# UCSD-Comp-Imaging/Nerf-Simple

Hardware: NVIDIA B200
Metric: rays/sec (64 samples/ray) render (higher is better)
Workload: dtype bf16

## Files before the change

nerf_simple_b200/csrc/mlp_chain.cuh:

```cuda
constexpr uint32_t kC_A = 0, kC_E = 2 * kABytes, kC_W = kC_E + 2 * kEBytes;
constexpr int kCStages = 4;
constexpr uint32_t kCStageBytes = 16384;
constexpr uint32_t kC_Bar = kC_W + kCStages * kCStageBytes;
constexpr uint32_t kC_Bias = kC_Bar + 256;
constexpr uint32_t kCSmemLaunch = kC_Bias + 2 * 1024;
constexpr int kCThreads = 640;
constexpr int kCProducerWarp = 16, kCMmaWarp = 17, kCStoreWarp0 = 18;
constexpr uint32_t kB_WFull = 0, kB_WPeer = 32, kB_WEmpty = 64, kB_Act = 96, kB_Acc = 112, kB_Tmem = 128, kB_Written = 136,
                   kB_StoreFree = 152;

struct TileCtx {
  int64_t tile;
  int slot;
  int half;
  int part;
  uint32_t r;
  uint32_t rowoff;
  uint32_t r7s;
  uint32_t a_img, e_img, t_lane;
  uint32_t b_img;
  const float* gf;
};
__device__ __forceinline__ uint32_t sw_off(const TileCtx& c, uint32_t kb, uint32_t j) {
  return kb * 16384u + c.rowoff + ((j << 4) ^ c.r7s);
}

__device__ __forceinline__ void slot_barrier(int slot) {
  asm volatile("bar.sync %0, 256;" ::"r"(slot + 1) : "memory");
}

#ifdef NB200_DEV
constexpr bool kDevBuild = true;
#else
constexpr bool kDevBuild = false;
#endif
struct SlabC { int src, kb, n, ksteps, both_a; };
constexpr int kSchedFwd = 0, kSchedBwd = 1, kSchedFwd3 = 2, kSchedFwdFold = 3;
constexpr int kSchedBwd3 = 4;
__host__ __device__ constexpr int sched_fwd_slabs(int l) { return l == 0 ? 1 : ((l == 5 || l == 9) ? 5 : 4); }
__host__ __device__ constexpr SlabC sched_fwd_slab(int l, int s) {
  return l == 0 ? SlabC{1, 0, 256, 4, 0}
                : (l == 9 ? (s < 4 ? SlabC{0, s, 128, 4, 0} : SlabC{1, 0, 128, 2, 0})
                          : (s < 4 ? SlabC{0, s, 256, 4, 0} : SlabC{1, 0, 256, 4, 0}));
}
template <int kSched> __host__ __device__ constexpr bool sched_is_bwd() { return kSched == kSchedBwd || kSched == kSchedBwd3; }
template <int kSched> __host__ __device__ constexpr int sched_slabs(int l) {
  return kSched == kSchedBwd3 ? 2 * (l == 0 ? 2 : 4)
         : kSched == kSchedFwd ? sched_fwd_slabs(l)
                             : (kSched == kSchedFwdFold ? sched_fwd_slabs(l >= 8 ? 9 : l) : (kSched == kSchedBwd ? (l == 0 ? 2 : 4) : 2 * sched_fwd_slabs(l)));
}
template <int kSched> __host__ __device__ constexpr SlabC sched_slab(int l, int s) {
  if (kSched == kSchedFwd) return sched_fwd_slab(l, s);
  if (kSched == kSchedFwdFold) return sched_fwd_slab(l >= 8 ? 9 : l, s);
  if (kSched == kSchedBwd) return SlabC{0, s, 256, 4, 0};
  if (kSched == kSchedBwd3) return SlabC{0, s >> 1, 256, 4, (s & 1) ? 0 : 1};
  SlabC c = sched_fwd_slab(l, s >> 1);
  c.both_a = (s & 1) ? 0 : 1;
  return c;
}

struct MmaRing { uint32_t stage, phase; };

template <int kSched> __host__ __device__ constexpr int sched_class_rep(int l) {
  return sched_is_bwd<kSched>() ? (l == 0 ? 0 : 1) : ((l == 0 || l == 5 || l == 9) ? l : ((kSched == kSchedFwdFold && l == 8) ? 9 : 1));
}

template <class Epi, int L, int S>
__device__ __forceinline__ void issue_slab(uint32_t smem_base, uint32_t bar, uint32_t tmem_base, uint64_t desc_hi, uint32_t slot,
                                           bool replay, bool release, MmaRing& r) {
  constexpr SlabC sc = sched_slab<Epi::kSched>(L, S);
  constexpr int NS = sched_slabs<Epi::kSched>(L);
  if (!replay) {
    mbar_wait(bar + kB_WFull + 8 * r.stage, r.phase, 400);
    tc_fence_after();
  }
  const uint32_t a_addr = smem_base + (sc.src ? kC_E + slot * kEBytes : kC_A + slot * kABytes + (uint32_t)sc.kb * 16384u);
  const uint64_t adesc = desc_hi | (uint64_t)((a_addr >> 4) & 0x3FFFu);
  const uint64_t bdesc = desc_hi | (uint64_t)(((smem_base + kC_W + r.stage * kCStageBytes) >> 4) & 0x3FFFu);
  constexpr uint32_t idesc = umma_idesc_bf16(256, sc.n, 0, 0);
// ... 96 lines not shown
    c.half = (warp >> 2) & 1;
    c.part = warp >> 2;
    c.r = (uint32_t)(warp & 3) * 32u + (uint32_t)lane;
    c.rowoff = c.r * 128u;
    c.r7s = (c.r & 7u) << 4;
    c.a_img = smem_base + kC_A + slot * kABytes;
    c.e_img = smem_base + kC_E + slot * kEBytes;
    c.t_lane = tmem_base + (((uint32_t)(warp & 3) * 32u) << 16) + (uint32_t)slot * 256u;
    c.b_img = smem_base + kC_Bias + (uint32_t)slot * 1024u;
    c.gf = reinterpret_cast<const float*>(p.packed + (Epi::kSched == kSchedFwd3 || Epi::kSched == kSchedBwd3 ? c_layout.f32_off3 : c_layout.f32_off));
    const uint32_t act_remote = mapa_shared(bar + kB_Act + 8 * slot, 0);
    uint32_t acc_parity = 0, free_parity = 0;
    typename Epi::State st;
    bool first_step = true;
    long long t_epi = 0, t_accw = 0, t_pro = 0, t_reclaim = 0, t_after = 0, t_stage = 0;
    auto publish = [&](bool to_mma) {
      fence_proxy_async_smem();
      tc_fence_before();
      __syncwarp();
      if (lane == 0) {
        if (Epi::kBulkStore) mbar_arrive(bar + kB_Written + 8 * slot);
        if (to_mma) mbar_arrive_cluster(act_remote);
      }
    };
    const uint32_t bias_t = threadIdx.x & 255u;
    auto fetch_bias = [&](int l) -> float { return Epi::kStageBias ? __ldg(c.gf + kF32Bias + Epi::bias_row(l) * 256 + (int)bias_t) : 0.f; };
    auto stage_bias = [&](float v) {
      if (!Epi::kStageBias) return;
      if (Epi::kSlots == 2) slot_barrier(slot); else asm volatile("bar.sync 1, 512;" ::: "memory");
      if (Epi::kSlots == 2 || threadIdx.x < 256u) asm volatile("st.shared.f32 [%0], %1;" ::"r"(c.b_img + bias_t * 4u), "f"(v) : "memory");
      if (Epi::kSlots == 2) slot_barrier(slot); else asm volatile("bar.sync 1, 512;" ::: "memory");
    };
    auto reclaim = [&]() {
      if (Epi::kBulkStore && !first_step) {
        mbar_wait(bar + kB_StoreFree + 8 * slot, free_parity, 500);
        free_parity ^= 1;
      }
      first_step = false;
    };
    Epi::init_slot(c);
    for (int64_t k = slot; k < my_pt; k += Epi::kSlots) {
      c.tile = 2 * (cid + k * C) + rank;
      if (Epi::kReverseTiles) c.tile = 2 * (PT - 1 - (cid + k * C)) + rank;
      reclaim();
      long long tq0 = 0;
      if constexpr (Epi::kHasDbg && kDevBuild) tq0 = clock64();
      const float bias0 = fetch_bias(0);
      Epi::begin_tile(p, st, c);
      publish(true);
      stage_bias(bias0);
      if constexpr (Epi::kHasDbg && kDevBuild) t_pro += clock64() - tq0;
      for (int l = 0; l < Epi::kNumLayers; ++l) {
        Epi::prefetch(p, st, c, l);
        if constexpr (Epi::kHasDbg && kDevBuild) tq0 = clock64();
        mbar_wait(bar + kB_Acc + 8 * slot, acc_parity, 100 + l);
        acc_parity ^= 1;
        tc_fence_after();
        long long tq1 = 0;
        if constexpr (Epi::kHasDbg && kDevBuild) { tq1 = clock64(); t_accw += tq1 - tq0; }
        reclaim();
        if constexpr (Epi::kHasDbg && kDevBuild) t_reclaim += clock64() - tq1;
        const float bias_next = fetch_bias(l + 1 < Epi::kNumLayers ? l + 1 : l);
        Epi::layer(p, st, c, l);
        if (Epi::kBulkStore || l + 1 < Epi::kNumLayers) publish(l + 1 < Epi::kNumLayers);
        if constexpr (Epi::kHasDbg && kDevBuild) {
          const long long tq2 = clock64();
          t_epi += tq2 - tq1;
          if ((p.dbg & 8) && threadIdx.x == 0 && rank == 0 && p.dbg_counters) {
            atomicAdd(p.dbg_counters + 16 + l, (unsigned long long)(tq2 - tq1));
            atomicAdd(p.dbg_counters + 32 + l, (unsigned long long)(tq1 - tq0));
          }
        }
        long long tq3 = 0;
        if constexpr (Epi::kHasDbg && kDevBuild) tq3 = clock64();
        if (l + 1 < Epi::kNumLayers) stage_bias(bias_next);
        long long tq4 = 0;
        if constexpr (Epi::kHasDbg && kDevBuild) { tq4 = clock64(); t_stage += tq4 - tq3; }
        Epi::after_publish(p, st, c, l);
        if constexpr (Epi::kHasDbg && kDevBuild) t_after += clock64() - tq4;
      }
    }
    if constexpr (Epi::kHasDbg && kDevBuild) {
      if ((p.dbg & 8) && threadIdx.x == 0 && rank == 0 && p.dbg_counters) {
        atomicAdd(p.dbg_counters + 4, (unsigned long long)t_epi);
        atomicAdd(p.dbg_counters + 5, (unsigned long long)t_accw);
        atomicAdd(p.dbg_counters + 6, (unsigned long long)t_pro);
        atomicAdd(p.dbg_counters + 12, (unsigned long long)t_reclaim);
        atomicAdd(p.dbg_counters + 13, (unsigned long long)t_stage);
        atomicAdd(p.dbg_counters + 14, (unsigned long long)t_after);
      }
    }
    if (Epi::kBulkStore && !first_step) mbar_wait(bar + kB_StoreFree + 8 * slot, free_parity, 501);
  } else if (warp == kCProducerWarp) {
    if (lane == 0) {
      uint32_t stage = 0, phase = 0;
      long long t_pempty = 0;
      for (int64_t pr = 0; pr * Epi::kSlots < my_pt; ++pr) {
        const int nslots = (Epi::kSlots == 2 && my_pt - 2 * pr >= 2) ? 2 : 1;
        int s0 = 0;
        for (int l = 0; l < Epi::kNumLayers; ++l) {
          int s1 = s0;
          while (!slabs[s1].last) ++s1;
          const int reps = (nslots == 2 && s1 - s0 + 1 <= kCStages) ? 1 : nslots;
          for (int rep = 0; rep < reps; ++rep) {
// ... 105 lines not shown
  float f;
  int64_t ray_begin;
};
constexpr int kInCamera = 2;

__device__ __forceinline__ void load_ray_chain(const FwdEpiParams& p, int64_t ray, float (&o)[6]) {
  if (p.in_mode == kInCamera) {
    camera_ray(p.poses, p.H, p.W, p.f, p.ray_begin + ray, o);
  } else {
    const float2* q = reinterpret_cast<const float2*>(p.in0 + ray * 6);
    const float2 a = __ldg(q), b = __ldg(q + 1), c = __ldg(q + 2);
    o[0] = a.x; o[1] = a.y; o[2] = b.x; o[3] = b.y; o[4] = c.x; o[5] = c.y;
  }
}

template <bool kRender>
__device__ __forceinline__ void load_query_chain(const FwdEpiParams& p, int64_t m, float v[6], float& t) {
  if (!kRender && p.in_mode == NB200_IN_POINTS) {
    const float2* q = reinterpret_cast<const float2*>(p.in0 + m * 6);
    const float2 a = __ldg(q), b = __ldg(q + 1), c = __ldg(q + 2);
    v[0] = a.x; v[1] = a.y; v[2] = b.x; v[3] = b.y; v[4] = c.x; v[5] = c.y;
    t = 0.f;
  } else {
    const int64_t ray = p.nshift >= 0 ? (m >> p.nshift) : m / p.N;
    float o[6];
    if (kRender) {
      load_ray_chain(p, ray, o);
      t = p.sampler ? philox_sample_depth(m, (int)(m - ray * p.N), p.N, p.tn, p.tf, p.seed, p.offset) : __ldg(p.in1 + m);
    } else {
      const float2* q = reinterpret_cast<const float2*>(p.in0 + ray * 6);
      const float2 a = __ldg(q), b = __ldg(q + 1), c = __ldg(q + 2);
      o[0] = a.x; o[1] = a.y; o[2] = b.x; o[3] = b.y; o[4] = c.x; o[5] = c.y;
      t = __ldg(p.in1 + m);
    }
    const float dx = o[3], dy = o[4], dz = o[5];
    v[0] = __fadd_rn(o[0], __fmul_rn(dx, t));
    v[1] = __fadd_rn(o[1], __fmul_rn(dy, t));
    v[2] = __fadd_rn(o[2], __fmul_rn(dz, t));
    const float inv = 1.0f / sqrtf(fmaf(dz, dz, fmaf(dy, dy, dx * dx)));
    v[3] = dx * inv; v[4] = dy * inv; v[5] = dz * inv;
  }
}

template <int S>
__device__ __forceinline__ void composite_staged_ray(const FwdEpiParams& p, uint32_t stage_o, uint32_t stage_t, int ray_local,
                                                     int64_t ray, int lane) {
  constexpr int N = 32 * S;
  float4 o[S];
  float t[S];
  const uint32_t row0 = (uint32_t)(ray_local * N + lane * S);
#pragma unroll
  for (int j = 0; j < S; ++j) {
    asm volatile("ld.shared.v4.f32 {%0,%1,%2,%3}, [%4];" : "=f"(o[j].x), "=f"(o[j].y), "=f"(o[j].z), "=f"(o[j].w) : "r"(stage_o + (row0 + j) * 16u));
    asm volatile("ld.shared.f32 %0, [%1];" : "=f"(t[j]) : "r"(stage_t + (row0 + j) * 4u));
  }
// ... 115 lines not shown
    load_bias16(c, cbase + (q + 1) * 16, bq);
    tmem_ld_wait();
    if (q + 2 < 8) tmem_ld16(c.t_lane + cbase + (q + 2) * 16, a0);
    epi_cols16<kRelu, kSigma, kSave>(c, a1, cbase + (q + 1) * 16, bq, sigma);
  }
}
template <bool kRelu, bool kSigma, bool kSave>
__device__ __forceinline__ void epi_hidden(const TileCtx& c, float& sigma) {
  if (c.half == 0) epi_hidden_h<kRelu, kSigma, kSave, 0>(c, sigma);
  else epi_hidden_h<kRelu, kSigma, kSave, 1>(c, sigma);
}
#ifdef NB_PROBE_NOLDTM
#undef tmem_ld16
#endif

template <bool kSave, bool kRender = false, bool kFold = false>
struct FwdEpi {
  static_assert(!(kSave && kRender), "the fused render kernel is inference only");
  using Params = FwdEpiParams;
  static constexpr bool kHasDbg = true;
  static constexpr bool kBulkStore = kSave;
  static constexpr int kSched = kFold ? kSchedFwdFold : kSchedFwd;
  static constexpr bool kStageBias = true;
  static constexpr int kSlots = 2;
  static constexpr int kNumLayers = kFold ? kNumFoldLayers : kNumMmaLayers;
  static constexpr bool kReverseTiles = false;
  __device__ static constexpr int ml_of(int l) { return (kFold && l == 8) ? 9 : l; }
  __device__ static constexpr int bias_row(int l) { return (kFold && l == 8) ? kFoldBiasRow : l; }
  struct State {
    float v[6];
    float sigma;
    float t;
    int64_t m_raw;
    bool row_valid;
  };
  __device__ static const SlabDesc* slabs() { return kFold ? c_layout.fwdf : c_layout.fwd; }
  __device__ static void init_slot(const TileCtx&) {}

  __device__ static void prefetch(const Params&, State&, const TileCtx&, int) {}

  __device__ static void after_publish(const Params& p, State& st, const TileCtx& c, int l) {
    const int ml = ml_of(l);
    if (ml == 5) {
      if (c.half == 0) encode_row<kLd, 0, 2>(st.v + 3, c.e_img, c.r, nullptr);
      else encode_row<kLd, 2, 4>(st.v + 3, c.e_img, c.r, nullptr);
#pragma unroll
      for (uint32_t i = threadIdx.x & 255u; i < kTabFloats; i += 256u) {
        const float v = __ldg(c.gf + (i < kTabWC1 ? kF32WSig + (int)i
                                                  : (i < kTabBC1 ? kF32WC1 + (int)(i - kTabWC1) : (i < kTabBSig ? kF32BC1 + (int)(i - kTabBC1) : kF32BSig))));
        asm volatile("st.shared.f32 [%0], %1;" ::"r"(c.e_img + tab_off(i)), "f"(v) : "memory");
      }
    }
    if (!kSave || ml < 0 || ml == 8) return;
    const int64_t T = p.num_tiles;
    if (ml < 8) {
      uint8_t* row = p.saved + mask_tensor_off(ml, T) + (size_t)c.tile * 4096 + ((size_t)(c.half * 128) + c.r) * 16;
      uint32_t m[4];
#pragma unroll
      for (int q = 0; q < 4; ++q) {
        const uint32_t kb = (uint32_t)(c.half * 2 + (q >> 1)), j0 = (uint32_t)(q & 1) * 4u;
// ... 19 lines not shown
          uint32_t w0, w1, w2, w3;
          asm volatile("ld.shared.v4.b32 {%0,%1,%2,%3}, [%4];" : "=r"(w0), "=r"(w1), "=r"(w2), "=r"(w3)
                       : "r"(c.a_img + sw_off(c, (uint32_t)c.half, (uint32_t)(q * 4 + j))));
          add_pair_flags(f[j >> 1], w0, 4 * (j & 1)); add_pair_flags(f[j >> 1], w1, 4 * (j & 1) + 1);
          add_pair_flags(f[j >> 1], w2, 4 * (j & 1) + 2); add_pair_flags(f[j >> 1], w3, 4 * (j & 1) + 3);
        }
        m[q] = fold_mask16(f[0]) | (fold_mask16(f[1]) << 16);
      }
      *reinterpret_cast<uint2*>(row) = make_uint2(m[0], m[1]);
    }
  }

  __device__ static void begin_tile(const Params& p, State& st, const TileCtx& c) {
    st.m_raw = c.tile * kTileM + c.r;
    st.row_valid = st.m_raw < p.M;
    load_query_chain<kRender>(p, st.row_valid ? st.m_raw : p.M - 1, st.v, st.t);
    st.sigma = 0.f;
    if (c.half == 0) encode_row<kLp, 0, 4>(st.v, c.e_img, c.r, nullptr);
    else encode_row<kLp, 4, 8>(st.v, c.e_img, c.r, nullptr);
  }

  __device__ static void store_tile(const Params& p, const TileCtx& c, int l) {
    const int64_t T = p.num_tiles;
    const int ml = ml_of(l);
    if (ml == -1) tma_bulk_s2g(p.saved + saved_tensor_off(10, T) + (size_t)c.tile * 16384, c.e_img, 16384);
    else if (ml < 9) tma_bulk_s2g(p.saved + saved_tensor_off(ml, T) + (size_t)c.tile * 65536, c.a_img, 65536);
    else tma_bulk_s2g(p.saved + saved_tensor_off(9, T) + (size_t)c.tile * 32768, c.a_img, 32768);
    if (ml == 6) tma_bulk_s2g(p.saved + saved_tensor_off(11, T) + (size_t)c.tile * 16384, c.e_img, 16384);
  }

  __device__ static void layer(const Params& p, State& st, const TileCtx& c, int l) {
    const int ml = ml_of(l);
    if (ml < 9) {
      if (ml == 7) epi_hidden<true, true, kSave>(c, st.sigma);
      else if (ml == 8) epi_hidden<false, false, kSave>(c, st.sigma);
      else epi_hidden<true, false, kSave>(c, st.sigma);
    } else {
      float rgb[3] = {0.f, 0.f, 0.f};
#pragma unroll 1
      for (int q = 0; q < 2; ++q) {
        const int col0 = c.half * 64 + q * 32;
        uint32_t a[32];
        tmem_ld32(c.t_lane + col0, a);
        tmem_ld_wait();
#pragma unroll
        for (int j = 0; j < 4; ++j) {
          float x[8], b[8];
          asm volatile("ld.shared.v4.f32 {%0,%1,%2,%3}, [%4];" : "=f"(b[0]), "=f"(b[1]), "=f"(b[2]), "=f"(b[3]) : "r"(c.b_img + (uint32_t)(col0 + 8 * j) * 4u));
          asm volatile("ld.shared.v4.f32 {%0,%1,%2,%3}, [%4];" : "=f"(b[4]), "=f"(b[5]), "=f"(b[6]), "=f"(b[7]) : "r"(c.b_img + (uint32_t)(col0 + 8 * j + 4) * 4u));
#pragma unroll
          for (int e = 0; e < 8; ++e) x[e] = fmaxf(__uint_as_float(a[8 * j + e]) + b[e], 0.f);
#pragma unroll
          for (int k = 0; k < 3; ++k) {
            const float4 w0 = tab_ld4(c.e_img, kTabWC1 + (uint32_t)(k * 128 + col0 + 8 * j)), w1 = tab_ld4(c.e_img, kTabWC1 + (uint32_t)(k * 128 + col0 + 8 * j + 4));
            rgb[k] = fmaf(x[0], w0.x, rgb[k]); rgb[k] = fmaf(x[1], w0.y, rgb[k]); rgb[k] = fmaf(x[2], w0.z, rgb[k]); rgb[k] = fmaf(x[3], w0.w, rgb[k]);
            rgb[k] = fmaf(x[4], w1.x, rgb[k]); rgb[k] = fmaf(x[5], w1.y, rgb[k]); rgb[k] = fmaf(x[6], w1.z, rgb[k]); rgb[k] = fmaf(x[7], w1.w, rgb[k]);
          }
          if (kSave) {
            const uint32_t w0 = pack_bf16x2(x[0], x[1]), w1 = pack_bf16x2(x[2], x[3]), w2 = pack_bf16x2(x[4], x[5]),
                           w3 = pack_bf16x2(x[6], x[7]);
            st_shared_v4(c.a_img + sw_off(c, (uint32_t)c.half, (uint32_t)(q * 4 + j)), w0, w1, w2, w3);
          }
        }
      }
// ... 53 lines not shown
#pragma unroll
    for (int e = 0; e < 4; ++e) split_hi_lo(f[8 * j + 2 * e], f[8 * j + 2 * e + 1], h[e], l[e]);
    st_shared_v4(img_hi + sw128_off(r, j), h[0], h[1], h[2], h[3]);
    st_shared_v4(img_lo + sw128_off(r, j), l[0], l[1], l[2], l[3]);
  }
}

__device__ __forceinline__ uint32_t relu_bit(int col_in_step) { return 1u << ((col_in_step >> 1) + 8 * (col_in_step & 1)); }

template <bool kSave>
struct FwdEpi3 {
  using Params = FwdEpiParams;
  static constexpr bool kHasDbg = false;
  static constexpr bool kBulkStore = kSave;
  static constexpr int kSched = kSchedFwd3;
  static constexpr bool kStageBias = true;
  static constexpr int kSlots = 1;
  static constexpr int kNumLayers = kNumMmaLayers;
  static constexpr bool kReverseTiles = false;
  struct State {
    float v[6];
    float sigma;
    int64_t m_raw;
    bool row_valid;
  };
  __device__ static const SlabDesc* slabs() { return c_layout.fwd3; }
  __device__ static constexpr int bias_row(int l) { return l; }
  __device__ static void init_slot(const TileCtx&) {}
  __device__ static void prefetch(const Params&, State&, const TileCtx&, int) {}
  __device__ static void after_publish(const Params&, State&, const TileCtx&, int) {}
// ... 142 lines not shown
      asm volatile("bar.sync 1, 512;" ::: "memory");
    }
  }
};

#ifndef NB_DG_L2HINT
#define NB_DG_L2HINT 2
#endif
template <bool kFold>
struct DgradEpi {
  using Params = BwdParams;
  static constexpr bool kHasDbg = false;
  static constexpr bool kBulkStore = true;
  static constexpr int kSched = kSchedBwd;
  static constexpr bool kStageBias = false;
  static constexpr int kSlots = 2;
  static constexpr int kNumLayers = kFold ? 8 : 9;
  static constexpr int kBl0 = kFold ? 2 : 1;
  static constexpr bool kReverseTiles = true;
  struct State { float4 g; uint4 mask; };
  __device__ static const SlabDesc* slabs() { return kFold ? c_layout.bwdf : c_layout.bwd; }
  __device__ static constexpr int bias_row(int l) { return l; }
  __device__ static void after_publish(const Params&, State&, const TileCtx&, int) {}
  __device__ static void init_slot(const TileCtx& c) {
    for (uint32_t i = threadIdx.x & 255u; i < 640u; i += 256u)
      asm volatile("st.shared.f32 [%0], %1;" ::"r"(c.e_img + i * 4u), "f"(__ldg(c.gf + (i < 256u ? kF32WSig + (int)i : kF32WC1 + (int)(i - 256u)))) : "memory");
    slot_barrier(c.slot);
  }
  __device__ static __forceinline__ float4 head_ld4(const TileCtx& c, uint32_t i) {
    float4 v;
// ... 93 lines not shown

  __device__ static void layer(const Params&, State& st, const TileCtx& c, int l) {
    const int bl = l + kBl0;
    if (bl == 1) layer_t<false, false>(st, c);
    else if (bl == 2) layer_t<true, true>(st, c);
    else layer_t<true, false>(st, c);
  }
};

struct DgradEpi3 {
  using Params = BwdParams;
  static constexpr bool kHasDbg = false;
  static constexpr bool kBulkStore = true;
  static constexpr int kSched = kSchedBwd3;
  static constexpr bool kStageBias = false;
  static constexpr int kSlots = 1;
  static constexpr int kNumLayers = 9;
  static constexpr bool kReverseTiles = true;
  struct State { float4 g; uint2 mask; };
  __device__ static const SlabDesc* slabs() { return c_layout.bwd3; }
  __device__ static constexpr int bias_row(int l) { return l; }
  __device__ static void after_publish(const Params&, State&, const TileCtx&, int) {}
  __device__ static void init_slot(const TileCtx& c) {
    for (uint32_t i = threadIdx.x; i < 640u; i += 512u)
      asm volatile("st.shared.f32 [%0], %1;" ::"r"(c.e_img + i * 4u), "f"(__ldg(c.gf + (i < 256u ? kF32WSig + (int)i : kF32WC1 + (int)(i - 256u)))) : "memory");
    asm volatile("bar.sync 1, 512;" ::: "memory");
  }
  __device__ static __forceinline__ float4 head_ld4(const TileCtx& c, uint32_t i) {
    float4 v;
    asm volatile("ld.shared.v4.f32 {%0,%1,%2,%3}, [%4];" : "=f"(v.x), "=f"(v.y), "=f"(v.z), "=f"(v.w) : "r"(c.e_img + i * 4u));
// ... 90 lines not shown
```

nerf_simple_b200/csrc/mlp_tc.cu:

```cuda
#include <cuda.h>
#include <stdlib.h>
#include <string.h>

#include <mutex>
#include <type_traits>
#include <utility>

#include "common.cuh"
#include "stream_common.cuh"
#include "tc_common.cuh"

namespace nb200 {
using namespace tc;

constexpr int kNumMmaLayers = 10;
constexpr int kMaxSlabs = 48;
constexpr int kNumFoldLayers = kNumMmaLayers - 1;
constexpr int kLayerFold = 100;
constexpr int kFoldBiasRow = 10;

struct SlabDesc {
  uint32_t off;
  uint32_t bytes;
  uint16_t n;
// ... 21 lines not shown
  SlabDesc bwd[kMaxSlabs];
  int num_fwdf;
  SlabDesc fwdf[kMaxSlabs];
  int num_bwdf;
  SlabDesc bwdf[kMaxSlabs];
  int num_fold;
  SlabDesc fold[8];
  uint32_t f32_off;
  uint32_t total_bytes;
  int num_fwd3;
  SlabDesc fwd3[2 * kMaxSlabs];
  uint32_t f32_off3;
  uint32_t total_bytes3;
  int num_bwd3;
  SlabDesc bwd3[2 * kMaxSlabs];
};
constexpr int kF32Bias = 0, kF32WSig = 2816, kF32BSig = 3072, kF32WC1 = 3076, kF32BC1 = 3460,
              kF32Floats = 3520;
constexpr int kF32Wf = kF32Floats, kF32WgT = kF32Wf + 128 * 256, kF32Wc0g = kF32WgT + 256 * 256, kF32Bg = kF32Wc0g + 128 * 256,
              kF32FloatsFold = kF32Bg + 256;

__constant__ __align__(16) PackedLayout c_layout;
static PackedLayout h_layout;
static bool h_layout_built = false;

constexpr int kMaxDevices = 64;
struct DeviceState { bool layout_uploaded, attr_fwd, attr_render, attr_bwd, attr_x3, attr_bwd3; int arch; };
static DeviceState g_dev[kMaxDevices];
static std::mutex g_mu;
static int current_device(int* dev) {
// ... 57 lines not shown
  }
  h_layout.num_bwd = t.s;
  LayoutBuilder f;
  f.arr = h_layout.fold; f.off = t.off; f.s = 0;
  for (int kb = 0; kb < 4; ++kb) f.add(9, kLayerFold, 0, 128, kb * 64, 64, kHidden, 0, kb, 4);
  for (int kb = 0; kb < 2; ++kb) f.add(2, kLayerFold, 1, 256, kb * 64, 64, kHidden, 0, kb, 4);
  h_layout.num_fold = f.s;
  {
    int n = 0;
    for (int i = 0; i < h_layout.num_fwd; ++i)
      if (h_layout.fwd[i].ml < 8) h_layout.fwdf[n++] = h_layout.fwd[i];
    for (int kb = 0; kb < 4; ++kb) h_layout.fwdf[n++] = h_layout.fold[kb];
    h_layout.fwdf[n - 4].first = 1;
    h_layout.fwdf[n++] = h_layout.fwd[h_layout.num_fwd - 1];
    h_layout.num_fwdf = n;
    n = 0;
    for (int kb = 0; kb < 2; ++kb) h_layout.bwdf[n++] = h_layout.fold[4 + kb];
    h_layout.bwdf[0].first = 1; h_layout.bwdf[1].last = 1;
    for (int i = 0; i < h_layout.num_bwd; ++i)
      if (h_layout.bwd[i].ml >= 3) h_layout.bwdf[n++] = h_layout.bwd[i];
    h_layout.num_bwdf = n;
  }
  h_layout.f32_off = f.off;
  h_layout.total_bytes = f.off + kF32FloatsFold * (uint32_t)sizeof(float);
  LayoutBuilder x;
  x.arr = h_layout.fwd3; x.off = 0; x.s = 0;
  for (int i = 0; i < h_layout.num_fwd; ++i) {
    const SlabDesc& f = h_layout.fwd[i];
    for (int lo = 0; lo < 2; ++lo) {
      x.add(f.ml, f.layer, 0, f.n, f.wcol0, f.kvalid, f.ldw, f.src, f.kb, f.ksteps, lo, lo ? 0 : 1);
// ... 193 lines not shown
__host__ __device__ __forceinline__ size_t mask_tensor_off(int t, int64_t num_tiles) {
  return (kSavedDataTileBytes + (size_t)t * 4096) * (size_t)num_tiles;
}
__host__ __device__ __forceinline__ size_t saved_tensor_off(int t, int64_t num_tiles) {
  const size_t per_tile = t < 9 ? (size_t)t * 65536 : (t == 9 ? 9 * 65536 : (t == 10 ? 9 * 65536 + 32768 : 9 * 65536 + 49152));
  return per_tile * (size_t)num_tiles;
}
__host__ __device__ __forceinline__ size_t saved_tile_bytes(int t) {
  return t < 9 ? 65536 : (t == 9 ? 32768 : 16384);
}
constexpr size_t kSavedTileBytes3 = 2 * kSavedDataTileBytes + kMaskTileBytes;
__host__ __device__ __forceinline__ size_t mask_tensor_off3(int t, int64_t num_tiles) {
  return (2 * kSavedDataTileBytes + (size_t)t * 4096) * (size_t)num_tiles;
}

template <int L, int J0, int J1>
__device__ __forceinline__ void encode_row(const float* x, uint32_t img_base, uint32_t r, uint8_t* gsave) {
  float f[64];
#pragma unroll
  for (int i = 0; i < 64; ++i) f[i] = 0.f;
#pragma unroll
  for (int c = 0; c < 3; ++c) {
    f[c] = x[c];
    float s, co;
    sincosf(x[c], &s, &co);
#pragma unroll
    for (int i = 0; i < L; ++i) {
      f[3 + c * 2 * L + 2 * i] = s;
      f[3 + c * 2 * L + 2 * i + 1] = co;
      const float s2 = 2.f * s * co;
      co = fmaf(-2.f * s, s, 1.f);
      s = s2;
    }
  }
#pragma unroll
  for (int j = J0; j < J1; ++j) {
    const uint32_t w0 = pack_bf16x2(f[8 * j], f[8 * j + 1]), w1 = pack_bf16x2(f[8 * j + 2], f[8 * j + 3]),
                   w2 = pack_bf16x2(f[8 * j + 4], f[8 * j + 5]), w3 = pack_bf16x2(f[8 * j + 6], f[8 * j + 7]);
    st_shared_v4(img_base + sw128_off(r, j), w0, w1, w2, w3);
    if (gsave) *reinterpret_cast<uint4*>(gsave + sw128_off(r, j)) = make_uint4(w0, w1, w2, w3);
  }
}

#include "mlp_tc_bwd.cuh"
#include "mlp_chain.cuh"

template <int kSched>
static bool schedule_matches(const SlabDesc* tab, int num, int layers) {
  int i = 0;
// ... 2 lines not shown
    for (int k = 0; k < ns; ++k, ++i) {
      if (i >= num) return false;
      const SlabC c = sched_slab<kSched>(l, k);
      const SlabDesc& d = tab[i];
      if (d.src != c.src || d.kb != c.kb || d.n != c.n || d.ksteps != c.ksteps || ((d.flags & kSlabBothA) != 0) != (c.both_a != 0) ||
          (d.first != 0) != (k == 0) || (d.last != 0) != (k == ns - 1) || d.bytes != (uint32_t)c.n * 128u)
        return false;
    }
  }
  return i == num;
}
static bool check_schedules() {
  return schedule_matches<kSchedFwd>(h_layout.fwd, h_layout.num_fwd, kNumMmaLayers) &&
         schedule_matches<kSchedBwd>(h_layout.bwd, h_layout.num_bwd, 9) &&
         schedule_matches<kSchedFwdFold>(h_layout.fwdf, h_layout.num_fwdf, kNumFoldLayers) &&
         schedule_matches<kSchedBwd>(h_layout.bwdf, h_layout.num_bwdf, 8) &&
         schedule_matches<kSchedFwd3>(h_layout.fwd3, h_layout.num_fwd3, kNumMmaLayers) &&
         schedule_matches<kSchedBwd3>(h_layout.bwd3, h_layout.num_bwd3, 9);
}

size_t tc_packed_bytes(int x3) {
  std::lock_guard<std::mutex> lock(g_mu);
  ensure_host_layout();
  return x3 ? h_layout.total_bytes3 : h_layout.total_bytes;
}
static int64_t train_tiles(int64_t M) { return (ceil_div64(M, kTileM) + 1) & ~(int64_t)1; }
size_t tc_saved_bytes(int64_t M) { return (size_t)train_tiles(M) * kSavedTileBytes; }
constexpr int kPadPitchWide = 320, kPadPitchX = 64;
constexpr size_t kPadC0 = 0, kPadSkip = kPadC0 + 128 * kPadPitchWide, kPadL00 = kPadSkip + 256 * kPadPitchWide,
                 kPadFoldS = kPadL00 + 256 * kPadPitchX,
// ... 139 lines not shown
}

int tc_forward(int in_mode, const float* in0, const float* in1, int64_t M, int N, const void* packed,
               float* out, void* saved, void*, size_t, int fold, cudaStream_t s) {
  NB_TRY_RC(check_arch());
  NB_TRY_RC(ensure_layout());
  NB_TRY_RC(ensure_attr(&DeviceState::attr_fwd, []() -> int {
    NB_CUDA_CHECK(cudaFuncSetAttribute(chain_kernel<FwdEpi<false>>, cudaFuncAttributeMaxDynamicSharedMemorySize,
                                       (int)kCSmemLaunch));
    NB_CUDA_CHECK(cudaFuncSetAttribute(chain_kernel<FwdEpi<true>>, cudaFuncAttributeMaxDynamicSharedMemorySize,
                                       (int)kCSmemLaunch));
    NB_CUDA_CHECK(cudaFuncSetAttribute(chain_kernel<FwdEpi<false, false, true>>, cudaFuncAttributeMaxDynamicSharedMemorySize,
                                       (int)kCSmemLaunch));
    NB_CUDA_CHECK(cudaFuncSetAttribute(chain_kernel<FwdEpi<true, false, true>>, cudaFuncAttributeMaxDynamicSharedMemorySize,
                                       (int)kCSmemLaunch));
    return NB200_OK;
  }));
  const int64_t T = saved ? train_tiles(M) : ceil_div64(M, kTileM);
  FwdEpiParams p;
  TmapPair tm;
  NB_TRY_RC(get_tmaps(packed, &tm));
  p.tmap128 = tm.m128; p.tmap64 = tm.m64;
  p.dbg = 0;
  p.dbg_counters = nullptr;
#ifdef NB200_DEV
  { const char* e = getenv("NB200_DBG"); p.dbg = e ? atoi(e) : 0; }
  if (p.dbg & 8) {
    static unsigned long long* ctr = nullptr;
    if (!ctr) { cudaMalloc(&ctr, 512); cudaMemset(ctr, 0, 512); }
    unsigned long long h[64];
    cudaMemcpy(h, ctr, 512, cudaMemcpyDeviceToHost);
    printf("nb200 dbg: mma-warp cycles wait_act=%llu total=%llu | epilogue warp 0: layers=%llu wait_acc=%llu prologue=%llu | producer wait_empty=%llu | epilogue warp 0: reclaim (inside layers)=%llu stage_bias=%llu after_publish=%llu\n",
           h[0], h[3], h[4], h[5], h[6], h[7], h[12], h[13], h[14]);
    printf("nb200 dbg: epilogue warp 0 per layer, busy | wait_acc (share of total):");
    for (int l = 0; l < 10; ++l) printf(" L%d %.1f|%.1f", l, 100.0 * (double)h[16 + l] / (double)(h[3] ? h[3] : 1), 100.0 * (double)h[32 + l] / (double)(h[3] ? h[3] : 1));
    printf("\n");
    cudaMemset(ctr, 0, 512);
    p.dbg_counters = ctr;
  }
#endif
  p.in_mode = in_mode; p.in0 = in0; p.in1 = in1; p.M = M; p.N = N;
  p.nshift = (N > 0 && (N & (N - 1)) == 0) ? __builtin_ctz((unsigned)N) : -1;
  p.packed = reinterpret_cast<const uint8_t*>(packed);
  p.out = out; p.saved = reinterpret_cast<uint8_t*>(saved);
  p.num_tiles = T;
  const int grid = chain_grid(T);
  if (saved && fold)
    chain_kernel<FwdEpi<true, false, true>><<<grid, kCThreads, kCSmemLaunch, s>>>(p);
  else if (saved)
    chain_kernel<FwdEpi<true>><<<grid, kCThreads, kCSmemLaunch, s>>>(p);
  else if (fold)
    chain_kernel<FwdEpi<false, false, true>><<<grid, kCThreads, kCSmemLaunch, s>>>(p);
  else
    chain_kernel<FwdEpi<false>><<<grid, kCThreads, kCSmemLaunch, s>>>(p);
  NB_LAUNCH_CHECK("chain_kernel<FwdEpi>");
  return NB200_OK;
}

static int chain_grid_x3(int64_t T) {
  const int64_t PT = (T + 1) / 2, maxc = sm_count() / 2;
  return (int)(2 * (PT < maxc ? PT : maxc));
}

int tc_forward_x3(int in_mode, const float* in0, const float* in1, int64_t M, int N, const void* packed, float* out,
                  void* saved, cudaStream_t s) {
// ... 21 lines not shown
  else chain_kernel<FwdEpi3<false>><<<grid, kCThreads, kCSmemLaunch, s>>>(p);
  NB_LAUNCH_CHECK("chain_kernel<FwdEpi3>");
  return NB200_OK;
}

int tc_render(const float* rays, const float* poses, int H, int W, float f, int64_t ray_begin, const float* ts, uint64_t seed,
              uint64_t offset, int64_t B, int N, float tn, float tf, const void* packed, float* rgb, float* disp, float* acc,
              int fold, cudaStream_t s) {
  NB_TRY_RC(check_arch());
  NB_TRY_RC(ensure_layout());
  NB_TRY_RC(ensure_attr(&DeviceState::attr_render, []() -> int {
    NB_CUDA_CHECK(cudaFuncSetAttribute(chain_kernel<FwdEpi<false, true>>, cudaFuncAttributeMaxDynamicSharedMemorySize,
                                       (int)kCSmemLaunch));
    NB_CUDA_CHECK(cudaFuncSetAttribute(chain_kernel<FwdEpi<false, true, true>>, cudaFuncAttributeMaxDynamicSharedMemorySize,
                                       (int)kCSmemLaunch));
    return NB200_OK;
  }));
  const int64_t M = B * N, T = ceil_div64(M, kTileM);
  FwdEpiParams p;
  memset(&p, 0, sizeof(p));
  TmapPair tm;
  NB_TRY_RC(get_tmaps(packed, &tm));
  p.tmap128 = tm.m128; p.tmap64 = tm.m64;
  p.in_mode = rays ? NB200_IN_RAYS : kInCamera; p.in0 = rays; p.in1 = ts; p.M = M; p.N = N;
  p.nshift = (N > 0 && (N & (N - 1)) == 0) ? __builtin_ctz((unsigned)N) : -1;
  p.packed = reinterpret_cast<const uint8_t*>(packed);
  p.num_tiles = T;
  p.rgb = rgb; p.disp = disp; p.acc = acc; p.B = B;
  p.sampler = ts ? 0 : 1; p.seed = seed; p.offset = offset; p.tn = tn; p.tf = tf;
  p.poses = poses; p.H = H; p.W = W; p.f = f; p.ray_begin = ray_begin;
  if (fold) chain_kernel<FwdEpi<false, true, true>><<<chain_grid(T), kCThreads, kCSmemLaunch, s>>>(p);
  else chain_kernel<FwdEpi<false, true>><<<chain_grid(T), kCThreads, kCSmemLaunch, s>>>(p);
  NB_LAUNCH_CHECK("chain_kernel<FwdEpi<render>>");
  return NB200_OK;
}

static void wgrad_item(WItem& w, const uint8_t* ds, const uint8_t* sv, int64_t T, float* pad, float* const* G, int dt, int st,
                       int layer, int ldw, int col0, int ncols, int nrows, bool bias) {
  w.a_ptr = ds + delta_tensor_off(dt, T);
  w.a_tile_bytes = dt == 0 ? 32768u : 65536u;
  w.a_chunks = dt == 0 ? 2 : 4;
  w.b_ptr = sv + saved_tensor_off(st, T);
  w.b_tile_bytes = (uint32_t)saved_tile_bytes(st);
  w.b_chunks = st >= 10 ? 1 : 4;
  w.n_mma = st >= 10 ? 64 : 256;
  w.dW = G[2 * layer]; w.db = bias ? G[2 * layer + 1] : nullptr;
// ... 171 lines not shown
```

Measured before the change: 20.03 million.

## Fold per-ray view-direction term into colour-layer bias for folded inference

Adds a ray-bias mode for the folded forward chain. Within a tile all samples share a ray direction, so the view-direction encoding's contribution to the colour layer is computed once per ray in scalar code and added to the bias. That drops the extra K-slab MMA and the direction encoding per sample. It also prefetches the next tile's ray and t values during the last layer in the non-render path, and adds debug timing for tile boundaries. In exchange the bias is now per ray, with two rays per 128-row tile when N is 64. The path is limited to N of 64 or 128, and the dot product is done on CUDA cores with bf16-rounded inputs.

```diff
diff --git a/nerf_simple_b200/csrc/mlp_chain.cuh b/nerf_simple_b200/csrc/mlp_chain.cuh
--- a/nerf_simple_b200/csrc/mlp_chain.cuh
+++ b/nerf_simple_b200/csrc/mlp_chain.cuh
@@ -19,6 +19,8 @@
   uint32_t r7s;
   uint32_t a_img, e_img, t_lane;
   uint32_t b_img;
+  bool first_tile;
+  int64_t next_tile;
   const float* gf;
 };
 __device__ __forceinline__ uint32_t sw_off(const TileCtx& c, uint32_t kb, uint32_t j) {
@@ -37,6 +39,7 @@
 struct SlabC { int src, kb, n, ksteps, both_a; };
 constexpr int kSchedFwd = 0, kSchedBwd = 1, kSchedFwd3 = 2, kSchedFwdFold = 3;
 constexpr int kSchedBwd3 = 4;
+constexpr int kSchedFwdRay = 5;
 __host__ __device__ constexpr int sched_fwd_slabs(int l) { return l == 0 ? 1 : ((l == 5 || l == 9) ? 5 : 4); }
 __host__ __device__ constexpr SlabC sched_fwd_slab(int l, int s) {
   return l == 0 ? SlabC{1, 0, 256, 4, 0}
@@ -47,11 +50,13 @@
 template <int kSched> __host__ __device__ constexpr int sched_slabs(int l) {
   return kSched == kSchedBwd3 ? 2 * (l == 0 ? 2 : 4)
          : kSched == kSchedFwd ? sched_fwd_slabs(l)
+         : kSched == kSchedFwdRay ? (l >= 8 ? 4 : sched_fwd_slabs(l))
                              : (kSched == kSchedFwdFold ? sched_fwd_slabs(l >= 8 ? 9 : l) : (kSched == kSchedBwd ? (l == 0 ? 2 : 4) : 2 * sched_fwd_slabs(l)));
 }
 template <int kSched> __host__ __device__ constexpr SlabC sched_slab(int l, int s) {
   if (kSched == kSchedFwd) return sched_fwd_slab(l, s);
   if (kSched == kSchedFwdFold) return sched_fwd_slab(l >= 8 ? 9 : l, s);
+  if (kSched == kSchedFwdRay) return l >= 8 ? SlabC{0, s, 128, 4, 0} : sched_fwd_slab(l, s);
   if (kSched == kSchedBwd) return SlabC{0, s, 256, 4, 0};
   if (kSched == kSchedBwd3) return SlabC{0, s >> 1, 256, 4, (s & 1) ? 0 : 1};
   SlabC c = sched_fwd_slab(l, s >> 1);
@@ -62,7 +67,8 @@
 struct MmaRing { uint32_t stage, phase; };
 
 template <int kSched> __host__ __device__ constexpr int sched_class_rep(int l) {
-  return sched_is_bwd<kSched>() ? (l == 0 ? 0 : 1) : ((l == 0 || l == 5 || l == 9) ? l : ((kSched == kSchedFwdFold && l == 8) ? 9 : 1));
+  return sched_is_bwd<kSched>() ? (l == 0 ? 0 : 1)
+                                : ((l == 0 || l == 5 || l == 9) ? l : (((kSched == kSchedFwdFold || kSched == kSchedFwdRay) && l == 8) ? 9 : 1));
 }
 
 template <class Epi, int L, int S>
@@ -189,6 +195,7 @@
     typename Epi::State st;
     bool first_step = true;
     long long t_epi = 0, t_accw = 0, t_pro = 0, t_reclaim = 0, t_after = 0, t_stage = 0;
+    long long t_bnd = 0, t_last_end = -1, n_bnd = 0;
     auto publish = [&](bool to_mma) {
       fence_proxy_async_smem();
       tc_fence_before();
@@ -199,7 +206,12 @@
       }
     };
     const uint32_t bias_t = threadIdx.x & 255u;
-    auto fetch_bias = [&](int l) -> float { return Epi::kStageBias ? __ldg(c.gf + kF32Bias + Epi::bias_row(l) * 256 + (int)bias_t) : 0.f; };
+    auto fetch_bias = [&](int l) -> float {
+      if constexpr (Epi::kRayBias) {
+        if (l == Epi::kNumLayers - 1) return st.u;
+      }
+      return Epi::kStageBias ? __ldg(c.gf + kF32Bias + Epi::bias_row(l) * 256 + (int)bias_t) : 0.f;
+    };
     auto stage_bias = [&](float v) {
       if (!Epi::kStageBias) return;
       if (Epi::kSlots == 2) slot_barrier(slot); else asm volatile("bar.sync 1, 512;" ::: "memory");
@@ -213,16 +225,21 @@
       }
       first_step = false;
     };
+    auto tile_of = [&](int64_t k) -> int64_t { return 2 * (Epi::kReverseTiles ? PT - 1 - (cid + k * C) : cid + k * C) + rank; };
     Epi::init_slot(c);
     for (int64_t k = slot; k < my_pt; k += Epi::kSlots) {
-      c.tile = 2 * (cid + k * C) + rank;
-      if (Epi::kReverseTiles) c.tile = 2 * (PT - 1 - (cid + k * C)) + rank;
+      c.tile = tile_of(k);
+      c.first_tile = k == slot;
+      c.next_tile = k + Epi::kSlots < my_pt ? tile_of(k + Epi::kSlots) : -1;
       reclaim();
       long long tq0 = 0;
       if constexpr (Epi::kHasDbg && kDevBuild) tq0 = clock64();
       const float bias0 = fetch_bias(0);
       Epi::begin_tile(p, st, c);
       publish(true);
+      if constexpr (Epi::kHasDbg && kDevBuild) {
+        if (t_last_end >= 0) { t_bnd += clock64() - t_last_end; ++n_bnd; }
+      }
       stage_bias(bias0);
       if constexpr (Epi::kHasDbg && kDevBuild) t_pro += clock64() - tq0;
       for (int l = 0; l < Epi::kNumLayers; ++l) {
@@ -241,6 +258,7 @@
         if constexpr (Epi::kHasDbg && kDevBuild) {
           const long long tq2 = clock64();
           t_epi += tq2 - tq1;
+          if (l + 1 == Epi::kNumLayers) t_last_end = tq2;
           if ((p.dbg & 8) && threadIdx.x == 0 && rank == 0 && p.dbg_counters) {
             atomicAdd(p.dbg_counters + 16 + l, (unsigned long long)(tq2 - tq1));
             atomicAdd(p.dbg_counters + 32 + l, (unsigned long long)(tq1 - tq0));
@@ -263,6 +281,8 @@
         atomicAdd(p.dbg_counters + 12, (unsigned long long)t_reclaim);
         atomicAdd(p.dbg_counters + 13, (unsigned long long)t_stage);
         atomicAdd(p.dbg_counters + 14, (unsigned long long)t_after);
+        atomicAdd(p.dbg_counters + 8, (unsigned long long)t_bnd);
+        atomicAdd(p.dbg_counters + 9, (unsigned long long)n_bnd);
       }
     }
     if (Epi::kBulkStore && !first_step) mbar_wait(bar + kB_StoreFree + 8 * slot, free_parity, 501);
@@ -398,6 +418,15 @@
   }
 }
 
+__device__ __forceinline__ void ray_query(const float* o, float t, float* v) {
+  const float dx = o[3], dy = o[4], dz = o[5];
+  v[0] = __fadd_rn(o[0], __fmul_rn(dx, t));
+  v[1] = __fadd_rn(o[1], __fmul_rn(dy, t));
+  v[2] = __fadd_rn(o[2], __fmul_rn(dz, t));
+  const float inv = 1.0f / sqrtf(fmaf(dz, dz, fmaf(dy, dy, dx * dx)));
+  v[3] = dx * inv; v[4] = dy * inv; v[5] = dz * inv;
+}
+
 template <bool kRender>
 __device__ __forceinline__ void load_query_chain(const FwdEpiParams& p, int64_t m, float v[6], float& t) {
   if (!kRender && p.in_mode == NB200_IN_POINTS) {
@@ -417,12 +446,7 @@
       o[0] = a.x; o[1] = a.y; o[2] = b.x; o[3] = b.y; o[4] = c.x; o[5] = c.y;
       t = __ldg(p.in1 + m);
     }
-    const float dx = o[3], dy = o[4], dz = o[5];
-    v[0] = __fadd_rn(o[0], __fmul_rn(dx, t));
-    v[1] = __fadd_rn(o[1], __fmul_rn(dy, t));
-    v[2] = __fadd_rn(o[2], __fmul_rn(dz, t));
-    const float inv = 1.0f / sqrtf(fmaf(dz, dz, fmaf(dy, dy, dx * dx)));
-    v[3] = dx * inv; v[4] = dy * inv; v[5] = dz * inv;
+    ray_query(o, t, v);
   }
 }
 
@@ -568,13 +592,15 @@
 #undef tmem_ld16
 #endif
 
-template <bool kSave, bool kRender = false, bool kFold = false>
+template <bool kSave, bool kRender = false, bool kFold = false, bool kRayBias_ = false>
 struct FwdEpi {
   static_assert(!(kSave && kRender), "the fused render kernel is inference only");
+  static_assert(!kRayBias_ || (kFold && !kSave), "the per-ray colour bias is an inference mode of the folded chain");
   using Params = FwdEpiParams;
   static constexpr bool kHasDbg = true;
   static constexpr bool kBulkStore = kSave;
-  static constexpr int kSched = kFold ? kSchedFwdFold : kSchedFwd;
+  static constexpr bool kRayBias = kRayBias_;
+  static constexpr int kSched = kRayBias ? kSchedFwdRay : (kFold ? kSchedFwdFold : kSchedFwd);
   static constexpr bool kStageBias = true;
   static constexpr int kSlots = 2;
   static constexpr int kNumLayers = kFold ? kNumFoldLayers : kNumMmaLayers;
@@ -585,19 +611,60 @@
     float v[6];
     float sigma;
     float t;
+    float u;
     int64_t m_raw;
     bool row_valid;
   };
-  __device__ static const SlabDesc* slabs() { return kFold ? c_layout.fwdf : c_layout.fwd; }
+  __device__ static const SlabDesc* slabs() { return kRayBias ? c_layout.fwdr : (kFold ? c_layout.fwdf : c_layout.fwd); }
   __device__ static void init_slot(const TileCtx&) {}
 
-  __device__ static void prefetch(const Params&, State&, const TileCtx&, int) {}
+  __device__ static void load_sample(const Params& p, State& st, int64_t m) {
+    load_ray_chain(p, m >> p.nshift, st.v);
+    st.t = __ldg(p.in1 + m);
+  }
+  __device__ static void prefetch(const Params& p, State& st, const TileCtx& c, int l) {
+    if constexpr (kRayBias && !kRender) {
+      if (ml_of(l) == 9 && c.next_tile >= 0) {
+        const int64_t m = c.next_tile * kTileM + c.r;
+        load_sample(p, st, m < p.M ? m : p.M - 1);
+      }
+    }
+  }
+
+  __device__ static float ray_bias(const Params& p, const TileCtx& c) {
+    const uint32_t bt = threadIdx.x & 255u, j = bt & 127u;
+    const int64_t nrays = p.M >> p.nshift;
+    int64_t ray = ((c.tile * kTileM) >> p.nshift) + (p.nshift == 6 ? (int64_t)(bt >> 7) : 0);
+    if (ray >= nrays) ray = nrays - 1;
+    float o[6], v[6];
+    load_ray_chain(p, ray, o);
+    ray_query(o, 0.f, v);
+    float f[64];
+    encode_feats<kLd>(v + 3, f);
+    const uint8_t* w = p.packed + c_layout.fwd[c_layout.num_fwd - 1].off;
+    float acc = 0.f;
+#pragma unroll
+    for (int q = 0; q < 4; ++q) {
+      const uint4 wq = __ldg(reinterpret_cast<const uint4*>(w + sw128_off(j, (uint32_t)q)));
+      const uint32_t ww[4] = {wq.x, wq.y, wq.z, wq.w};
+#pragma unroll
+      for (int e = 0; e < 4; ++e) {
+        const uint32_t fw = pack_bf16x2(f[8 * q + 2 * e], f[8 * q + 2 * e + 1]);
+        acc = fmaf(__uint_as_float(fw << 16), __uint_as_float(ww[e] << 16), acc);
+        acc = fmaf(__uint_as_float(fw & 0xFFFF0000u), __uint_as_float(ww[e] & 0xFFFF0000u), acc);
+      }
+    }
+    return __ldg(c.gf + kF32Bias + kFoldBiasRow * 256 + (int)j) + acc;
+  }
 
   __device__ static void after_publish(const Params& p, State& st, const TileCtx& c, int l) {
     const int ml = ml_of(l);
+    if (kRayBias && ml == 6) st.u = ray_bias(p, c);
     if (ml == 5) {
-      if (c.half == 0) encode_row<kLd, 0, 2>(st.v + 3, c.e_img, c.r, nullptr);
-      else encode_row<kLd, 2, 4>(st.v + 3, c.e_img, c.r, nullptr);
+      if (!kRayBias) {
+        if (c.half == 0) encode_row<kLd, 0, 2>(st.v + 3, c.e_img, c.r, nullptr);
+        else encode_row<kLd, 2, 4>(st.v + 3, c.e_img, c.r, nullptr);
+      }
 #pragma unroll
       for (uint32_t i = threadIdx.x & 255u; i < kTabFloats; i += 256u) {
         const float v = __ldg(c.gf + (i < kTabWC1 ? kF32WSig + (int)i
@@ -647,7 +714,12 @@
   __device__ static void begin_tile(const Params& p, State& st, const TileCtx& c) {
     st.m_raw = c.tile * kTileM + c.r;
     st.row_valid = st.m_raw < p.M;
-    load_query_chain<kRender>(p, st.row_valid ? st.m_raw : p.M - 1, st.v, st.t);
+    if constexpr (kRayBias && !kRender) {
+      if (c.first_tile) load_sample(p, st, st.row_valid ? st.m_raw : p.M - 1);
+      ray_query(st.v, st.t, st.v);
+    } else {
+      load_query_chain<kRender>(p, st.row_valid ? st.m_raw : p.M - 1, st.v, st.t);
+    }
     st.sigma = 0.f;
     if (c.half == 0) encode_row<kLp, 0, 4>(st.v, c.e_img, c.r, nullptr);
     else encode_row<kLp, 4, 8>(st.v, c.e_img, c.r, nullptr);
@@ -670,6 +742,7 @@
       else epi_hidden<true, false, kSave>(c, st.sigma);
     } else {
       float rgb[3] = {0.f, 0.f, 0.f};
+      const uint32_t b_row = c.b_img + ((kRayBias && p.nshift == 6 && c.r >= 64u) ? 512u : 0u);
 #pragma unroll 1
       for (int q = 0; q < 2; ++q) {
         const int col0 = c.half * 64 + q * 32;
@@ -679,8 +752,8 @@
 #pragma unroll
         for (int j = 0; j < 4; ++j) {
           float x[8], b[8];
-          asm volatile("ld.shared.v4.f32 {%0,%1,%2,%3}, [%4];" : "=f"(b[0]), "=f"(b[1]), "=f"(b[2]), "=f"(b[3]) : "r"(c.b_img + (uint32_t)(col0 + 8 * j) * 4u));
-          asm volatile("ld.shared.v4.f32 {%0,%1,%2,%3}, [%4];" : "=f"(b[4]), "=f"(b[5]), "=f"(b[6]), "=f"(b[7]) : "r"(c.b_img + (uint32_t)(col0 + 8 * j + 4) * 4u));
+          asm volatile("ld.shared.v4.f32 {%0,%1,%2,%3}, [%4];" : "=f"(b[0]), "=f"(b[1]), "=f"(b[2]), "=f"(b[3]) : "r"(b_row + (uint32_t)(col0 + 8 * j) * 4u));
+          asm volatile("ld.shared.v4.f32 {%0,%1,%2,%3}, [%4];" : "=f"(b[4]), "=f"(b[5]), "=f"(b[6]), "=f"(b[7]) : "r"(b_row + (uint32_t)(col0 + 8 * j + 4) * 4u));
 #pragma unroll
           for (int e = 0; e < 8; ++e) x[e] = fmaxf(__uint_as_float(a[8 * j + e]) + b[e], 0.f);
 #pragma unroll
@@ -764,6 +837,7 @@
   static constexpr bool kHasDbg = false;
   static constexpr bool kBulkStore = kSave;
   static constexpr int kSched = kSchedFwd3;
+  static constexpr bool kRayBias = false;
   static constexpr bool kStageBias = true;
   static constexpr int kSlots = 1;
   static constexpr int kNumLayers = kNumMmaLayers;
@@ -936,6 +1010,7 @@
   static constexpr bool kBulkStore = true;
   static constexpr int kSched = kSchedBwd;
   static constexpr bool kStageBias = false;
+  static constexpr bool kRayBias = false;
   static constexpr int kSlots = 2;
   static constexpr int kNumLayers = kFold ? 8 : 9;
   static constexpr int kBl0 = kFold ? 2 : 1;
@@ -1059,6 +1134,7 @@
   static constexpr bool kBulkStore = true;
   static constexpr int kSched = kSchedBwd3;
   static constexpr bool kStageBias = false;
+  static constexpr bool kRayBias = false;
   static constexpr int kSlots = 1;
   static constexpr int kNumLayers = 9;
   static constexpr bool kReverseTiles = true;
diff --git a/nerf_simple_b200/csrc/mlp_tc.cu b/nerf_simple_b200/csrc/mlp_tc.cu
--- a/nerf_simple_b200/csrc/mlp_tc.cu
+++ b/nerf_simple_b200/csrc/mlp_tc.cu
@@ -59,6 +59,8 @@
   uint32_t total_bytes3;
   int num_bwd3;
   SlabDesc bwd3[2 * kMaxSlabs];
+  int num_fwdr;
+  SlabDesc fwdr[kMaxSlabs];
 };
 constexpr int kF32Bias = 0, kF32WSig = 2816, kF32BSig = 3072, kF32WC1 = 3076, kF32BC1 = 3460,
               kF32Floats = 3520;
@@ -146,6 +148,9 @@
     h_layout.fwdf[n - 4].first = 1;
     h_layout.fwdf[n++] = h_layout.fwd[h_layout.num_fwd - 1];
     h_layout.num_fwdf = n;
+    for (int i = 0; i + 1 < h_layout.num_fwdf; ++i) h_layout.fwdr[i] = h_layout.fwdf[i];
+    h_layout.num_fwdr = h_layout.num_fwdf - 1;
+    h_layout.fwdr[h_layout.num_fwdr - 1].last = 1;
     n = 0;
     for (int kb = 0; kb < 2; ++kb) h_layout.bwdf[n++] = h_layout.fold[4 + kb];
     h_layout.bwdf[0].first = 1; h_layout.bwdf[1].last = 1;
@@ -369,9 +374,8 @@
   return (2 * kSavedDataTileBytes + (size_t)t * 4096) * (size_t)num_tiles;
 }
 
-template <int L, int J0, int J1>
-__device__ __forceinline__ void encode_row(const float* x, uint32_t img_base, uint32_t r, uint8_t* gsave) {
-  float f[64];
+template <int L>
+__device__ __forceinline__ void encode_feats(const float* x, float (&f)[64]) {
 #pragma unroll
   for (int i = 0; i < 64; ++i) f[i] = 0.f;
 #pragma unroll
@@ -388,6 +392,11 @@
       s = s2;
     }
   }
+}
+template <int L, int J0, int J1>
+__device__ __forceinline__ void encode_row(const float* x, uint32_t img_base, uint32_t r, uint8_t* gsave) {
+  float f[64];
+  encode_feats<L>(x, f);
 #pragma unroll
   for (int j = J0; j < J1; ++j) {
     const uint32_t w0 = pack_bf16x2(f[8 * j], f[8 * j + 1]), w1 = pack_bf16x2(f[8 * j + 2], f[8 * j + 3]),
@@ -420,6 +429,7 @@
   return schedule_matches<kSchedFwd>(h_layout.fwd, h_layout.num_fwd, kNumMmaLayers) &&
          schedule_matches<kSchedBwd>(h_layout.bwd, h_layout.num_bwd, 9) &&
          schedule_matches<kSchedFwdFold>(h_layout.fwdf, h_layout.num_fwdf, kNumFoldLayers) &&
+         schedule_matches<kSchedFwdRay>(h_layout.fwdr, h_layout.num_fwdr, kNumFoldLayers) &&
          schedule_matches<kSchedBwd>(h_layout.bwdf, h_layout.num_bwdf, 8) &&
          schedule_matches<kSchedFwd3>(h_layout.fwd3, h_layout.num_fwd3, kNumMmaLayers) &&
          schedule_matches<kSchedBwd3>(h_layout.bwd3, h_layout.num_bwd3, 9);
@@ -589,6 +599,8 @@
                                        (int)kCSmemLaunch));
     NB_CUDA_CHECK(cudaFuncSetAttribute(chain_kernel<FwdEpi<true, false, true>>, cudaFuncAttributeMaxDynamicSharedMemorySize,
                                        (int)kCSmemLaunch));
+    NB_CUDA_CHECK(cudaFuncSetAttribute(chain_kernel<FwdEpi<false, false, true, true>>, cudaFuncAttributeMaxDynamicSharedMemorySize,
+                                       (int)kCSmemLaunch));
     return NB200_OK;
   }));
   const int64_t T = saved ? train_tiles(M) : ceil_div64(M, kTileM);
@@ -607,6 +619,8 @@
     cudaMemcpy(h, ctr, 512, cudaMemcpyDeviceToHost);
     printf("nb200 dbg: mma-warp cycles wait_act=%llu total=%llu | epilogue warp 0: layers=%llu wait_acc=%llu prologue=%llu | producer wait_empty=%llu | epilogue warp 0: reclaim (inside layers)=%llu stage_bias=%llu after_publish=%llu\n",
            h[0], h[3], h[4], h[5], h[6], h[7], h[12], h[13], h[14]);
+    printf("nb200 dbg: epilogue warp 0 tile boundary (last epilogue done -> next tile's act arrive): %llu cycles over %llu boundaries = %.0f per boundary\n",
+           h[8], h[9], (double)h[8] / (double)(h[9] ? h[9] : 1));
     printf("nb200 dbg: epilogue warp 0 per layer, busy | wait_acc (share of total):");
     for (int l = 0; l < 10; ++l) printf(" L%d %.1f|%.1f", l, 100.0 * (double)h[16 + l] / (double)(h[3] ? h[3] : 1), 100.0 * (double)h[32 + l] / (double)(h[3] ? h[3] : 1));
     printf("\n");
@@ -624,6 +638,8 @@
     chain_kernel<FwdEpi<true, false, true>><<<grid, kCThreads, kCSmemLaunch, s>>>(p);
   else if (saved)
     chain_kernel<FwdEpi<true>><<<grid, kCThreads, kCSmemLaunch, s>>>(p);
+  else if (fold && in_mode == NB200_IN_RAYS && (N == 64 || N == 128))
+    chain_kernel<FwdEpi<false, false, true, true>><<<grid, kCThreads, kCSmemLaunch, s>>>(p);
   else if (fold)
     chain_kernel<FwdEpi<false, false, true>><<<grid, kCThreads, kCSmemLaunch, s>>>(p);
   else
@@ -675,6 +691,8 @@
                                        (int)kCSmemLaunch));
     NB_CUDA_CHECK(cudaFuncSetAttribute(chain_kernel<FwdEpi<false, true, true>>, cudaFuncAttributeMaxDynamicSharedMemorySize,
                                        (int)kCSmemLaunch));
+    NB_CUDA_CHECK(cudaFuncSetAttribute(chain_kernel<FwdEpi<false, true, true, true>>, cudaFuncAttributeMaxDynamicSharedMemorySize,
+                                       (int)kCSmemLaunch));
     return NB200_OK;
   }));
   const int64_t M = B * N, T = ceil_div64(M, kTileM);
@@ -690,7 +708,8 @@
   p.rgb = rgb; p.disp = disp; p.acc = acc; p.B = B;
   p.sampler = ts ? 0 : 1; p.seed = seed; p.offset = offset; p.tn = tn; p.tf = tf;
   p.poses = poses; p.H = H; p.W = W; p.f = f; p.ray_begin = ray_begin;
-  if (fold) chain_kernel<FwdEpi<false, true, true>><<<chain_grid(T), kCThreads, kCSmemLaunch, s>>>(p);
+  if (fold && (N == 64 || N == 128)) chain_kernel<FwdEpi<false, true, true, true>><<<chain_grid(T), kCThreads, kCSmemLaunch, s>>>(p);
+  else if (fold) chain_kernel<FwdEpi<false, true, true>><<<chain_grid(T), kCThreads, kCSmemLaunch, s>>>(p);
   else chain_kernel<FwdEpi<false, true>><<<chain_grid(T), kCThreads, kCSmemLaunch, s>>>(p);
   NB_LAUNCH_CHECK("chain_kernel<FwdEpi<render>>");
   return NB200_OK;
```

Result: faster. 20.37 million, median of 6 (+1.7%).
